# rrahn/libspm

Hardware: AMD Instinct MI355X
Metric: Gbases/s scanned, Myers k<=3 |P|=100 (higher is better)
Workload: dtype u32

## Files before the change

libspm_amd/csrc/filter.hpp:

```cpp
#pragma once

#include "brute.hpp"
#include "common.hpp"
#include "filter_shared.hpp"
#include "pack.hpp"
#include "hd.hpp"

namespace spm_hip
{

struct survivor
{
    uint32_t key;
    uint32_t t_lo, t_hi;
    uint32_t pad;
};
constexpr uint32_t kSurvInvalid = 0xFFFFFFFFu;

struct band_rec
{
    uint32_t slot;
    uint32_t val;
    uint32_t seg;
    uint32_t band;
// ... 256 lines not shown
            uint32_t wu = w[0], pu = prev[0];
#pragma unroll
            for (int q = 1; q < NWD; ++q)
                if (u == q) {
                    wu = w[q];
                    pu = prev[q];
                }
            key = (d == 16 ? wu : alignbit(wu, pu, (uint32_t)(2 * d) & 31u)) & kmask;
            const uint64_t wpos = PK ? gbase + (uint64_t)(u >> 2) * 4096 + (uint64_t)lane * 64 + (uint64_t)(u & 3) * 16
                                     : gbase + (uint64_t)u * 1024 + (uint64_t)lane * 16;
            const int64_t ts = (int64_t)wpos - 16 + d;
            if (ts >= (int64_t)P.lo && (uint64_t)ts + P.key_len <= P.hi) {
                t = (uint64_t)ts;
                has = true;
            }
        }
        emit_survivors(P, has, key, t, lane, lds);
    }
}



__device__ __forceinline__ uint32_t anchor_select(uint32_t w, uint32_t prev, uint32_t c, uint32_t cm)
{
    const uint32_t C0 = (c & 3u) * 0x55555555u, M0 = (cm & 3u) * 0x55555555u;
    const uint32_t C1 = (c >> 2) * 0x55555555u, M1 = (cm >> 2) * 0x55555555u;
    const uint32_t X = alignbit(w, prev, 2);
    const uint32_t Y = alignbit(w, prev, 4);
    uint32_t t = ((X ^ C0) & M0) | ((Y ^ C1) & M1);
    t |= t >> 1;
    return ~t & 0x55555555u;
}

template <int NWD>
__device__ __forceinline__ void filter_words_anchored(const filter_params &P, const uint32_t (&w)[NWD], const uint32_t (&prev)[NWD],
                                                      uint64_t gbase, uint32_t lane, const uint32_t *lds)
{
    static_assert(NWD % 2 == 0 || NWD == 1, "words are taken in pairs");
    const uint16_t *fp_tab = reinterpret_cast<const uint16_t *>(lds);
    const uint16_t *disp_tab = reinterpret_cast<const uint16_t *>(reinterpret_cast<const uint8_t *>(lds) + P.chd_disp_off);
#pragma unroll
    for (int j = 0; j < NWD; j += 2) {
        uint32_t todo = anchor_select(w[j], prev[j], P.anchor_c, P.anchor_cm);
        if (j + 1 < NWD)
            todo |= anchor_select(w[j + 1 < NWD ? j + 1 : j], prev[j + 1 < NWD ? j + 1 : j], P.anchor_c, P.anchor_cm) << 1;
        while (__ballot(todo != 0) != 0) {
            const bool act = todo != 0;
            const uint32_t b = act ? (uint32_t)__ffs(todo) - 1u : 0u;
            todo &= todo - 1;
            const uint32_t u = b & 1u, d = (b >> 1) + 1u;
            const uint32_t wu = (j + 1 < NWD && u) ? w[j + 1 < NWD ? j + 1 : j] : w[j];
            const uint32_t pu = (j + 1 < NWD && u) ? prev[j + 1 < NWD ? j + 1 : j] : prev[j];
            const uint32_t key = (uint32_t)((((uint64_t)wu << 32) | pu) >> (2 * d));
            const uint32_t x = chd_hash(key).x;
            const uint32_t dsp = disp_tab[x >> P.chd_bucket_shift];
            const uint32_t slot = ((x >> 3) + dsp * ((key | 1u) & 0xFFFFFFu)) & P.chd_slot_mask;
            const uint32_t f = fp_tab[slot];
            const bool hit = act && ((f ^ key ^ (key >> 16)) & 0xFFFFu) == 0;
            if (__ballot(hit) != 0) {
                if (__builtin_amdgcn_readfirstlane(cand_chunk_of(P, lds)[5]) != 0)
                    return;
                const uint64_t wpos = gbase + (uint64_t)(j + u) * 1024 + (uint64_t)lane * 16;
                const int64_t ts = (int64_t)wpos - 16 + (int64_t)d;
                const bool has = hit && ts >= (int64_t)P.lo && (uint64_t)ts + P.key_len <= P.hi;
                emit_survivors(P, has, key, has ? (uint64_t)ts : 0, lane, lds);
            }
        }
    }
}


__device__ __forceinline__ void stream_stage(const filter_params &P, uint32_t *lds)
{
    for (uint32_t i = threadIdx.x; i < P.lds_words; i += blockDim.x)
        lds[i] = P.bitmap[i];
    if ((threadIdx.x & 63) == 0) {
        uint32_t *ck = lds + P.lds_words + kCandLdsSlot + kCandRec * (threadIdx.x >> 6);
        for (uint32_t i = 0; i < kCandRec; ++i)
            ck[i] = 0;
    }
    __syncthreads();
}

enum class span_draw
{
    run,
    idle,
    done,
};

__device__ __forceinline__ span_draw draw_span(const filter_params &P, uint32_t *lds, uint32_t lane, uint32_t wave_in_wg,
                                               uint32_t waves_per_wg, uint64_t n_spans, uint64_t &sp)
{
    if (P.dynamic == 1) {
        unsigned long long t = 0;
        if (lane == 0)
            t = atomicAdd(&P.counters[kCntSpanHead], 1ull);
        sp = uniform_u64(t);
        return sp >= n_spans ? span_draw::done : span_draw::run;
    }
    __syncthreads();
    if (threadIdx.x == 0) {
        const unsigned long long t = atomicAdd(&P.counters[kCntSpanHead], (unsigned long long)waves_per_wg);
        lds[P.lds_words] = (uint32_t)t;
        lds[P.lds_words + 1] = (uint32_t)(t >> 32);
    }
    __syncthreads();
    const uint64_t base = uniform_u64(((uint64_t)lds[P.lds_words + 1] << 32) | lds[P.lds_words]);
    if (base >= n_spans)
        return span_draw::done;
    sp = base + wave_in_wg;
    return sp >= n_spans ? span_draw::idle : span_draw::run;
}

template <int SIG>
__device__ __forceinline__ uint32_t span_carry_in(const filter_params &P, uint64_t span_base, uint32_t lane, uint32_t &carry_n)
{
    uint32_t carry_in = 0;
    carry_n = 0;
    if (span_base >= 16 && lane == 0) {
        const uint4 before = load_text16(P.text, span_base - 16, P.hi);
        carry_in = pack16_sig<SIG>(before, carry_n);
    }
    carry_n = __builtin_amdgcn_readfirstlane(carry_n);
    return __builtin_amdgcn_readfirstlane(carry_in);
}

__device__ __forceinline__ uint32_t span_carry_in(const filter_params &P, uint64_t span_base, uint32_t lane)
{
    uint32_t no_n;
    return span_carry_in<4>(P, span_base, lane, no_n);
}

__device__ __forceinline__ void pack_with_prev(const uint4 &cur, uint32_t lane, uint32_t &carry_in, uint32_t &w, uint32_t &prev)
{
    w = pack16(cur);
    prev = __builtin_amdgcn_update_dpp(0u, w, 0x138 , 0xF, 0xF, false);
    if (lane == 0)
        prev = carry_in;
    carry_in = __builtin_amdgcn_readlane(w, 63);
}

template <int S, int UU, int HV, int SIG, bool KM, bool AN = false>
__device__ __forceinline__ void filter_group(const filter_params &P, const uint4 (&cur)[UU], uint64_t gbase,
                                             uint32_t &carry_in, uint32_t &carry_n, uint32_t lane,
                                             const uint32_t *lds, uint32_t idx_mask)
{
    uint32_t w[UU], prev[UU];
    uint32_t nv[SIG != 4 ? UU : 1];
#pragma unroll
    for (int u = 0; u < UU; ++u) {
        if constexpr (SIG == 4) {
            pack_with_prev(cur[u], lane, carry_in, w[u], prev[u]);
        } else {
            uint32_t nm = 0;
            w[u] = pack16_sig<SIG>(cur[u], nm);
            prev[u] = __builtin_amdgcn_update_dpp(0u, w[u], 0x138 , 0xF, 0xF, false);
            if (lane == 0)
                prev[u] = carry_in;
            carry_in = __builtin_amdgcn_readlane(w[u], 63);
            uint32_t np = __builtin_amdgcn_update_dpp(0u, nm, 0x138, 0xF, 0xF, false);
            if (lane == 0)
                np = carry_n;
            carry_n = __builtin_amdgcn_readlane(nm, 63);
            nv[u] = (nm << 16) | np;
        }
    }
    if constexpr (AN)
        filter_words_anchored<UU>(P, w, prev, gbase, lane, lds);
    else
        filter_words<S, UU, HV, SIG, false, KM>(P, w, prev, nv, gbase, lane, lds, idx_mask);
}

template <int S, int U, int HV, int SIG, bool KM, bool AN = false>
__global__ __launch_bounds__(((S == 1 && !KM && SIG == 4) || (S == 2 && U == 2)) ? 1024 : 512) void seed_filter_kernel(const filter_params P)
{
    extern __shared__ uint32_t lds[];
    stream_stage(P, lds);

    const uint32_t lane = threadIdx.x & 63;
    const uint32_t waves_per_wg = blockDim.x >> 6;
    const uint32_t wave_in_wg = (uint32_t)__builtin_amdgcn_readfirstlane(threadIdx.x >> 6);
    const uint32_t idx_mask = P.bitmap_words * 32 - 1;

    const stream_geometry G = stream_geometry_of(P.lo, P.hi, 1024, P.span_chunks);
    const uint64_t span = P.span_chunks;
    const uint8_t *lane_text = P.text + G.base0 + (uint64_t)lane * 16;

    uint64_t sp;
    for (;;) {
        const span_draw drawn = draw_span(P, lds, lane, wave_in_wg, waves_per_wg, G.n_spans, sp);
        if (drawn == span_draw::done)
            break;
        if (drawn == span_draw::idle)
            continue;
        const uint64_t c_begin = sp * span;
        const uint64_t c_end = c_begin + span < G.n_chunks ? c_begin + span : G.n_chunks;
        span_open(P, lds, lane, G.base0 + c_begin * 1024);
        uint32_t carry_n;
        uint32_t carry_in = span_carry_in<SIG>(P, G.base0 + c_begin * 1024, lane, carry_n);
        uint64_t ch = c_begin;
        const uint64_t whole_end = c_end < G.n_whole ? c_end : G.n_whole;
        const uint64_t fast_end = c_begin + (whole_end > c_begin ? (whole_end - c_begin) / U * U : 0);
        if (ch < fast_end) {
            uint4 nxt[U];
#pragma unroll
            for (int u = 0; u < U; ++u)
                nxt[u] = load16_stream(lane_text + (ch + u) * 1024);
            for (; ch < fast_end; ch += U) {
                uint4 cur[U];
#pragma unroll
                for (int u = 0; u < U; ++u)
                    cur[u] = nxt[u];
                const bool more = ch + U < fast_end;
                const uint64_t pf = more ? ch + U : ch;
                const uint64_t ustride = more ? 1024 : 0;
#pragma unroll
                for (int u = 0; u < U; ++u)
                    nxt[u] = load16_stream(lane_text + pf * 1024 + (uint64_t)u * ustride);
                if constexpr (S <= 2)
                    __builtin_amdgcn_sched_barrier(0);
                filter_group<S, U, HV, SIG, KM, AN>(P, cur, G.base0 + ch * 1024, carry_in, carry_n, lane, lds, idx_mask);
            }
        }
        for (; ch < c_end; ++ch) {
            uint4 one[1];
            one[0] = load_text16(P.text, (G.base0 + ch * 1024) | ((uint64_t)lane * 16), P.hi);
            filter_group<S, 1, HV, SIG, KM, AN>(P, one, G.base0 + ch * 1024, carry_in, carry_n, lane, lds, idx_mask);
        }
    }
    surv_close(P, cand_chunk_of(P, lds), lane);
}

constexpr uint32_t kDenseQueueCap = 192;
constexpr int kDenseBatches = 3;

template <int NP>
__device__ __forceinline__ uint32_t dense_select(const filter_params &P, uint32_t w, uint32_t prev)
{
    const uint32_t X = alignbit(w, prev, 2);
    const uint32_t Y = alignbit(w, prev, 4);
    uint32_t sel = 0;
#pragma unroll
    for (int i = 0; i < NP; ++i) {
        const uint32_t C0 = (P.pat_c[i] & 3u) * 0x55555555u, M0 = (P.pat_cm[i] & 3u) * 0x55555555u;
        const uint32_t C1 = (P.pat_c[i] >> 2) * 0x55555555u, M1 = (P.pat_cm[i] >> 2) * 0x55555555u;
        uint32_t t = ((X ^ C0) & M0) | ((Y ^ C1) & M1);
        t |= t >> 1;
        sel |= ~t;
    }
    return sel & 0x55555555u;
}

struct dense_queue
{
    uint32_t key[kDenseQueueCap];
    uint32_t off[kDenseQueueCap];
};

__device__ __forceinline__ void dense_drain(const filter_params &P, dense_queue &Q, uint32_t &qn, bool all, uint64_t span_base,
                                            uint32_t lane, const uint32_t *lds)
{
    while (qn >= 64 || (all && qn != 0)) {
        const uint32_t nb_full = qn >> 6;
        uint32_t nb = all ? (qn + 63) >> 6 : nb_full;
        nb = nb > (uint32_t)kDenseBatches ? (uint32_t)kDenseBatches : nb;
        uint32_t key[kDenseBatches], off[kDenseBatches];
        uint4 bk[kDenseBatches];
        bool v[kDenseBatches];
#pragma unroll
        for (int b = 0; b < kDenseBatches; ++b) {
            const int32_t e = (int32_t)qn - 64 * b - 1 - (int32_t)lane;
            v[b] = (uint32_t)b < nb && e >= 0;
            key[b] = 0;
            off[b] = 0;
            bk[b] = make_uint4(0, 0, 0, 0);
            if (v[b]) {
                key[b] = Q.key[e];
                off[b] = Q.off[e];
                bk[b] = P.buckets[dense_bucket(key[b], P.bucket_shift)];
            }
        }
        qn = qn > 64 * nb ? qn - 64 * nb : 0;
#pragma unroll
        for (int b = 0; b < kDenseBatches; ++b) {
            if ((uint32_t)b >= nb)
                break;
            const uint32_t f2 = dense_fp(key[b]) * 0x00010001u;
            const uint32_t x0 = bk[b].x ^ f2, x1 = bk[b].y ^ f2, x2 = bk[b].z ^ f2, x3 = bk[b].w ^ f2;
            const uint32_t z = ((x0 - 0x00010001u) & ~x0) | ((x1 - 0x00010001u) & ~x1) | ((x2 - 0x00010001u) & ~x2) |
                               ((x3 - 0x00010001u) & ~x3);
            const bool hit = v[b] && ((z & 0x80008000u) != 0 || (bk[b].w >> 16) == kDenseAcceptAll);
            if (__ballot(hit) != 0) {
                if (__builtin_amdgcn_readfirstlane(cand_chunk_of(P, lds)[5]) == 0) {
                    const int64_t ts = (int64_t)span_base + (int64_t)off[b] - 16;
                    const bool has = hit && ts >= (int64_t)P.lo && (uint64_t)ts + P.key_len <= P.hi;
                    emit_survivors(P, has, key[b], has ? (uint64_t)ts : 0, lane, lds);
                }
            }
        }
    }
}

template <int UU, int NP, int S, bool KM>
__device__ __forceinline__ void dense_group(const filter_params &P, const uint4 (&cur)[UU], uint64_t gbase, uint64_t span_base,
                                            uint32_t &carry_in, uint32_t lane, const uint32_t *lds, dense_queue &Q, uint32_t &qn)
{
    static_assert(UU % 2 == 0 || UU == 1, "words are taken in pairs");
    uint32_t w[UU], prev[UU];
#pragma unroll
    for (int u = 0; u < UU; ++u)
        pack_with_prev(cur[u], lane, carry_in, w[u], prev[u]);
    const uint32_t goff = (uint32_t)(gbase - span_base) + lane * 16;
#pragma unroll
    for (int j = 0; j < UU; j += 2) {
        constexpr bool pair = UU > 1;
        const uint32_t w0 = w[j], p0 = prev[j], w1 = w[pair ? j + 1 : j], p1 = prev[pair ? j + 1 : j];
        const uint32_t kmask = KM ? P.key_mask : 0xFFFFFFFFu;
        static_assert(kDenseBloomBits == 20, "the word address below takes bits 5..19 of the index");
        uint32_t pm = 0;
        if constexpr (S == 0) {
            uint32_t todo = dense_select<NP>(P, w0, p0);
            if (pair)
                todo |= dense_select<NP>(P, w1, p1) << 1;
            while (todo != 0) {
                const uint32_t b = (uint32_t)__ffs(todo) - 1u;
                todo &= todo - 1;
                const bool odd = (b & 1u) != 0;
                const uint64_t both = ((uint64_t)(odd ? w1 : w0) << 32) | (odd ? p1 : p0);
                const uint32_t key = (uint32_t)(both >> ((b & ~1u) + 2u));
                const uint32_t h = key ^ (key >> 13);
                const uint32_t word = *reinterpret_cast<const uint32_t *>(reinterpret_cast<const uint8_t *>(lds) + ((h >> 3) & 0x1FFFCu));
                pm |= __builtin_amdgcn_ubfe(word, h, 1) << b;
            }
        } else {
#pragma unroll
            for (int u = 0; u < (pair ? 2 : 1); ++u) {
#pragma unroll
                for (int d = S; d <= 16; d += S) {
                    const uint32_t wu = u ? w1 : w0, pu = u ? p1 : p0;
                    const uint32_t key = (d == 16 ? wu : alignbit(wu, pu, (2 * d) & 31)) & kmask;
                    const uint32_t h = key ^ (key >> 13);
                    const uint32_t word = *reinterpret_cast<const uint32_t *>(reinterpret_cast<const uint8_t *>(lds) + ((h >> 3) & 0x1FFFCu));
                    pm |= __builtin_amdgcn_ubfe(word, h, 1) << (2 * (d - 1) + u);
                }
            }
        }
        while (__ballot(pm != 0) != 0) {
            const bool pos = pm != 0;
            const uint32_t b = pos ? (uint32_t)__ffs(pm) - 1u : 0u;
            pm &= pm - 1;
            const bool odd = (b & 1u) != 0;
            const uint64_t both = ((uint64_t)(odd ? w1 : w0) << 32) | (odd ? p1 : p0);
            const uint32_t key = (uint32_t)(both >> ((b & ~1u) + 2u)) & kmask;
            const uint64_t mm = __ballot(pos);
            if (pos) {
                const uint32_t q = qn + __popcll(mm & ((1ull << lane) - 1));
                Q.key[q] = key;
                Q.off[q] = goff + (uint32_t)j * 1024u + (odd ? 1024u : 0u) + (b >> 1) + 1u;
            }
            qn += __popcll(mm);
            queue_sync();
            if (qn > kDenseQueueCap - 64)
                dense_drain(P, Q, qn, false, span_base, lane, lds);
        }
    }
}

template <int U, int NP, int S = 0, bool KM = false>
__global__ __launch_bounds__(1024) void seed_filter_dense_kernel(const filter_params P)
{
    extern __shared__ uint32_t lds[];
    stream_stage(P, lds);

    const uint32_t lane = threadIdx.x & 63;
    const uint32_t waves_per_wg = blockDim.x >> 6;
    const uint32_t wave_in_wg = (uint32_t)__builtin_amdgcn_readfirstlane(threadIdx.x >> 6);
    dense_queue &Q = *reinterpret_cast<dense_queue *>(lds + P.lds_words + kCandLdsSlot + kCandRec * 16 +
                                                      (sizeof(dense_queue) / 4) * wave_in_wg);
    uint32_t qn = 0;

    const stream_geometry G = stream_geometry_of(P.lo, P.hi, 1024, P.span_chunks);
    const uint64_t span = P.span_chunks;
    const uint8_t *lane_text = P.text + G.base0 + (uint64_t)lane * 16;

    uint64_t sp;
    for (;;) {
        const span_draw drawn = draw_span(P, lds, lane, wave_in_wg, waves_per_wg, G.n_spans, sp);
        if (drawn == span_draw::done)
            break;
        if (drawn == span_draw::idle)
            continue;
        const uint64_t c_begin = sp * span;
        const uint64_t c_end = c_begin + span < G.n_chunks ? c_begin + span : G.n_chunks;
        const uint64_t span_base = G.base0 + c_begin * 1024;
        span_open(P, lds, lane, span_base);
        uint32_t carry_in = span_carry_in(P, span_base, lane);
        uint64_t ch = c_begin;
        const uint64_t whole_end = c_end < G.n_whole ? c_end : G.n_whole;
        const uint64_t fast_end = c_begin + (whole_end > c_begin ? (whole_end - c_begin) / U * U : 0);
        if (ch < fast_end) {
            uint4 nxt[U];
#pragma unroll
            for (int u = 0; u < U; ++u)
                nxt[u] = load16_stream(lane_text + (ch + u) * 1024);
            for (; ch < fast_end; ch += U) {
                uint4 cur[U];
#pragma unroll
                for (int u = 0; u < U; ++u)
                    cur[u] = nxt[u];
                const bool more = ch + U < fast_end;
                const uint64_t pf = more ? ch + U : ch;
                const uint64_t ustride = more ? 1024 : 0;
#pragma unroll
                for (int u = 0; u < U; ++u)
                    nxt[u] = load16_stream(lane_text + pf * 1024 + (uint64_t)u * ustride);
                __builtin_amdgcn_sched_barrier(0);
                dense_group<U, NP, S, KM>(P, cur, G.base0 + ch * 1024, span_base, carry_in, lane, lds, Q, qn);
            }
        }
        for (; ch < c_end; ++ch) {
            uint4 one[1];
            one[0] = load_text16(P.text, G.base0 + ch * 1024 + (uint64_t)lane * 16, P.hi);
            dense_group<1, NP, S, KM>(P, one, G.base0 + ch * 1024, span_base, carry_in, lane, lds, Q, qn);
        }
        dense_drain(P, Q, qn, true, span_base, lane, lds);
    }
    surv_close(P, cand_chunk_of(P, lds), lane);
}

template <int S, int U2, int HV, bool KM>
__global__ __launch_bounds__(1024) void seed_filter_packed_kernel(const filter_params P, const uint4 *__restrict__ shadow)
{
    extern __shared__ uint32_t lds[];
    stream_stage(P, lds);

    constexpr int NWD = 4 * U2;
    const uint32_t lane = threadIdx.x & 63;
    const uint32_t waves_per_wg = blockDim.x >> 6;
    const uint32_t wave_in_wg = (uint32_t)__builtin_amdgcn_readfirstlane(threadIdx.x >> 6);
    const uint32_t idx_mask = P.bitmap_words * 32 - 1;

    const stream_geometry G = stream_geometry_of(P.lo, P.hi, 4096, P.span_chunks);
    const uint64_t span = P.span_chunks;
    const uint4 *lane_src = shadow + (G.base0 / 64) + lane;

    uint64_t sp;
    for (;;) {
        const span_draw drawn = draw_span(P, lds, lane, wave_in_wg, waves_per_wg, G.n_spans, sp);
        if (drawn == span_draw::done)
            break;
        if (drawn == span_draw::idle)
            continue;
        const uint64_t c_begin = sp * span;
        const uint64_t c_end = c_begin + span < G.n_chunks ? c_begin + span : G.n_chunks;
        const uint64_t fast_end = c_begin + (c_end - c_begin + U2 - 1) / U2 * U2;
        span_open(P, lds, lane, G.base0 + c_begin * 4096);
        uint32_t carry_in = 0;
        {
            const uint64_t first_word = (G.base0 + c_begin * 4096) / 16;
            if (first_word > 0 && lane == 0)
                carry_in = reinterpret_cast<const uint32_t *>(shadow)[first_word - 1];
            carry_in = __builtin_amdgcn_readfirstlane(carry_in);
        }
        uint4 nxt[U2];
#pragma unroll
        for (int u = 0; u < U2; ++u)
            nxt[u] = load16_stream(reinterpret_cast<const uint8_t *>(lane_src + (c_begin + u) * 64));
        for (uint64_t ch = c_begin; ch < fast_end; ch += U2) {
            uint4 cur[U2];
#pragma unroll
            for (int u = 0; u < U2; ++u)
                cur[u] = nxt[u];
            const bool more = ch + U2 < fast_end;
            const uint64_t pf = more ? ch + U2 : ch;
            const uint64_t ustride = more ? 64 : 0;
#pragma unroll
            for (int u = 0; u < U2; ++u)
                nxt[u] = load16_stream(reinterpret_cast<const uint8_t *>(lane_src + pf * 64 + (uint64_t)u * ustride));
            __builtin_amdgcn_sched_barrier(0);
            uint32_t w[NWD], prev[NWD];
            const uint32_t nv[1] = {0};
#pragma unroll
            for (int u = 0; u < U2; ++u) {
                w[4 * u + 0] = cur[u].x;
                w[4 * u + 1] = cur[u].y;
                w[4 * u + 2] = cur[u].z;
                w[4 * u + 3] = cur[u].w;
                uint32_t p0 = __builtin_amdgcn_update_dpp(0u, cur[u].w, 0x138 , 0xF, 0xF, false);
                if (lane == 0)
                    p0 = carry_in;
                carry_in = __builtin_amdgcn_readlane(cur[u].w, 63);
                prev[4 * u + 0] = p0;
                prev[4 * u + 1] = cur[u].x;
                prev[4 * u + 2] = cur[u].y;
                prev[4 * u + 3] = cur[u].z;
            }
            filter_words<S, NWD, HV, 4, true, KM>(P, w, prev, nv, G.base0 + ch * 4096, lane, lds, idx_mask);
        }
    }
    surv_close(P, cand_chunk_of(P, lds), lane);
}

struct verify_params
{
    const uint8_t *text;
    uint64_t text_alloc;
    uint64_t ctx_begin;
    uint64_t scan_begin;
    uint64_t scan_end;
    uint64_t pos_offset;
    const band_rec *bands;
    const unsigned long long *counters;
    uint32_t band_counter;
    uint32_t preselected;
    uint64_t band_cap;
    ulonglong2 *band_tab;
    uint32_t table_mask, band_bits;
    uint32_t runs;
    const uint8_t *surplus;
    uint32_t Bw;
    uint32_t overlap;
    uint32_t max_m;
    const uint32_t *peq32;
    uint32_t sigma;
    uint32_t nw_table;
    uint32_t max_k;
    const int32_t *m;
    const int32_t *k;
    uint32_t report_begin;
    uint32_t max_span;
    uint32_t wave_text;
    unsigned long long *seen;
    uint32_t seen_mask;
    spm_hit *hits;
    unsigned long long *hit_counter;
    uint64_t hit_cap;
    unsigned long long *overflow;
    const uint64_t *seg_offsets;
    uint64_t n_segments;
    const uint32_t *seg_owned;
};

struct resolve_params
{
    const survivor *surv;
    unsigned long long *counters;
    uint64_t surv_cap;
    const pass_entry *passes;
    const uint4 *entries;
    uint32_t key_len;
    uint32_t flank_check;
    uint32_t pieces_check;
    const uint8_t *text;
    uint64_t text_alloc;
    const uint8_t *needle_ranks;
    const uint32_t *needle_offsets;
    const uint16_t *seed_q;
    const int32_t *m, *k;
    uint64_t hay_begin, hay_end;
    const uint64_t *seg_offsets;
    uint64_t n_segments;
    uint32_t Bw, overlap, max_m;
    uint32_t band_bits;
    ulonglong2 *band_tab;
    uint32_t table_mask;
    band_rec *bands;
    uint64_t band_cap;
    const uint32_t *needle_pk;
    const uint32_t *pk_offsets;
    uint32_t exact_hits;
    uint32_t report_begin;
    uint64_t scan_begin, scan_end;
    uint64_t pos_offset;
    const uint32_t *seg_owned;
    unsigned long long *seen;
    uint32_t seen_mask;
    spm_hit *hits;
    unsigned long long *hit_counter, *overflow;
    uint64_t hit_cap;
    uint32_t *table_poison;
};

__device__ __forceinline__ unsigned long long band_value(unsigned long long stored, bool counting)
{
    return counting ? (unsigned long long)(uint32_t)(stored + 1ull) : ~stored;
}
__device__ __forceinline__ void band_release(ulonglong2 *tab, uint32_t slot)
{
    tab[slot] = make_ulonglong2(kBandEmpty, ~0ull);
}

__device__ __forceinline__ uint4 load_bytes16(const uint8_t *p)
{
    uint4 v;
    __builtin_memcpy(&v, p, 16);
    return v;
}

__device__ __forceinline__ uint4 load_bytes16_guarded(const uint8_t *base, uint64_t idx, uint64_t limit)
{
    if (idx + 16 <= limit)
        return load_bytes16(base + idx);
    uint32_t w[4] = {0xFFFFFFFFu, 0xFFFFFFFFu, 0xFFFFFFFFu, 0xFFFFFFFFu};
    for (int b = 0; b < 16; ++b)
        if (idx + b < limit)
            w[b >> 2] = (w[b >> 2] & ~(0xFFu << (8 * (b & 3)))) | ((uint32_t)base[idx + b] << (8 * (b & 3)));
    return make_uint4(w[0], w[1], w[2], w[3]);
}

__device__ __forceinline__ uint32_t diff16(const uint4 a, const uint4 b, uint32_t n)
{
    const uint32_t d[4] = {a.x ^ b.x, a.y ^ b.y, a.z ^ b.z, a.w ^ b.w};
    uint32_t r = 0;
#pragma unroll
    for (uint32_t i = 0; i < 4; ++i) {
        const uint32_t have = n > 4 * i ? n - 4 * i : 0;
        const uint32_t mask = have >= 4 ? 0xFFFFFFFFu : (have == 0 ? 0u : (1u << (8 * have)) - 1);
        r |= d[i] & mask;
    }
    return r;
}

__device__ __forceinline__ bool seed_intact(const resolve_params &P, uint64_t t, uint32_t val, uint32_t r, uint32_t q_whole,
                                            int64_t hay_b, int64_t hay_e)
{
    if (!P.needle_ranks)
        return true;
    const uint32_t pat = val >> 11, x = val & 0x7FF;
    struct
    {
        uint32_t q;
    } sp{q_whole ? q_whole : P.seed_q[pat]};
    const uint32_t o = x - r;
    const int64_t ts = (int64_t)t - (int64_t)r;
    if (ts < hay_b || ts + (int64_t)sp.q > hay_e)
        return false;
    const uint8_t *nd = P.needle_ranks + P.needle_offsets[pat] + o;
    for (uint32_t i = 0; i < sp.q; i += 16) {
        const uint32_t n = sp.q - i < 16 ? sp.q - i : 16;
        if (diff16(load_bytes16_guarded(P.text, (uint64_t)ts + i, P.text_alloc), load_bytes16(nd + i), n))
            return false;
    }
    return true;
}

constexpr uint32_t kPieceRoundsShift = 21, kPieceMissingShift = 28;

__device__ __forceinline__ bool pieces_apply(const resolve_params &P, uint64_t t, uint32_t val, uint32_t m, uint32_t k, int64_t hay_b,
                                             int64_t hay_e)
{
    if (!P.pieces_check || k == 0 || k > 7 || m < 32)
        return false;
    const int64_t d = (int64_t)t - (int64_t)(val & 0x7FF);
    return d - (int64_t)k >= hay_b && d + (int64_t)(m + k) <= hay_e;
}

__device__ __forceinline__ uint32_t pieces_visit(const resolve_params &P, uint64_t t, uint32_t val, uint32_t &rng, uint32_t m, uint32_t k)
{
    const uint32_t pat = val >> 11, x = val & 0x7FF;
    const uint32_t n_rounds = m >> 4;
    uint32_t done = (rng >> kPieceRoundsShift) & 0x7F, missing = (rng >> kPieceMissingShift) & 7;
// ... 1126 lines not shown
```

Before: 6463.

## Batch dense survivor enqueue with a wave prefix sum and pair the bloom probes

The per-pair ballot loop that appended one hit per lane per iteration is replaced. Each lane now gathers presence masks for all word pairs, counts its hits, and uses a DPP wave prefix sum to get its write offset into the queue. All hits are then written in bulk, in chunks bounded by the remaining queue room. The S==0 selection loop also probes two candidate positions per iteration to expose more LDS-load parallelism. This is meant to cut the ballot and queue_sync rounds per group and keep lanes from idling on uneven hit counts, at the cost of more registers for the held masks and a more complex chunked drain loop.

```diff
diff --git a/libspm_amd/csrc/filter.hpp b/libspm_amd/csrc/filter.hpp
--- a/libspm_amd/csrc/filter.hpp
+++ b/libspm_amd/csrc/filter.hpp
@@ -582,36 +582,61 @@
     }
 }
 
+__device__ __forceinline__ uint32_t wave_prefix_sum(uint32_t v)
+{
+    v += __builtin_amdgcn_update_dpp(0u, v, 0x111 , 0xF, 0xF, false);
+    v += __builtin_amdgcn_update_dpp(0u, v, 0x112 , 0xF, 0xF, false);
+    v += __builtin_amdgcn_update_dpp(0u, v, 0x114 , 0xF, 0xF, false);
+    v += __builtin_amdgcn_update_dpp(0u, v, 0x118 , 0xF, 0xF, false);
+    v += __builtin_amdgcn_update_dpp(0u, v, 0x142 , 0xA, 0xF, false);
+    v += __builtin_amdgcn_update_dpp(0u, v, 0x143 , 0xC, 0xF, false);
+    return v;
+}
+
+__device__ __forceinline__ uint32_t dense_pair_key(uint32_t w0, uint32_t p0, uint32_t w1, uint32_t p1, uint32_t b)
+{
+    const bool odd = (b & 1u) != 0;
+    const uint64_t both = ((uint64_t)(odd ? w1 : w0) << 32) | (odd ? p1 : p0);
+    return (uint32_t)(both >> ((b & ~1u) + 2u));
+}
+
+__device__ __forceinline__ uint32_t dense_presence_word(const uint32_t *lds, uint32_t h)
+{
+    static_assert(kDenseBloomBits == 20, "the word address takes bits 5..19 of the index");
+    return *reinterpret_cast<const uint32_t *>(reinterpret_cast<const uint8_t *>(lds) + ((h >> 3) & 0x1FFFCu));
+}
+
 template <int UU, int NP, int S, bool KM>
 __device__ __forceinline__ void dense_group(const filter_params &P, const uint4 (&cur)[UU], uint64_t gbase, uint64_t span_base,
                                             uint32_t &carry_in, uint32_t lane, const uint32_t *lds, dense_queue &Q, uint32_t &qn)
 {
     static_assert(UU % 2 == 0 || UU == 1, "words are taken in pairs");
+    constexpr bool pair = UU > 1;
+    constexpr int NPM = pair ? UU / 2 : 1;
     uint32_t w[UU], prev[UU];
 #pragma unroll
     for (int u = 0; u < UU; ++u)
         pack_with_prev(cur[u], lane, carry_in, w[u], prev[u]);
     const uint32_t goff = (uint32_t)(gbase - span_base) + lane * 16;
+    const uint32_t kmask = KM ? P.key_mask : 0xFFFFFFFFu;
+    uint32_t pmv[NPM];
 #pragma unroll
     for (int j = 0; j < UU; j += 2) {
-        constexpr bool pair = UU > 1;
         const uint32_t w0 = w[j], p0 = prev[j], w1 = w[pair ? j + 1 : j], p1 = prev[pair ? j + 1 : j];
-        const uint32_t kmask = KM ? P.key_mask : 0xFFFFFFFFu;
-        static_assert(kDenseBloomBits == 20, "the word address below takes bits 5..19 of the index");
-        uint32_t pm = 0;
+        uint32_t m = 0;
         if constexpr (S == 0) {
             uint32_t todo = dense_select<NP>(P, w0, p0);
             if (pair)
                 todo |= dense_select<NP>(P, w1, p1) << 1;
             while (todo != 0) {
-                const uint32_t b = (uint32_t)__ffs(todo) - 1u;
+                const uint32_t b0 = (uint32_t)__ffs(todo) - 1u;
                 todo &= todo - 1;
-                const bool odd = (b & 1u) != 0;
-                const uint64_t both = ((uint64_t)(odd ? w1 : w0) << 32) | (odd ? p1 : p0);
-                const uint32_t key = (uint32_t)(both >> ((b & ~1u) + 2u));
-                const uint32_t h = key ^ (key >> 13);
-                const uint32_t word = *reinterpret_cast<const uint32_t *>(reinterpret_cast<const uint8_t *>(lds) + ((h >> 3) & 0x1FFFCu));
-                pm |= __builtin_amdgcn_ubfe(word, h, 1) << b;
+                const uint32_t b1 = todo != 0 ? (uint32_t)__ffs(todo) - 1u : b0;
+                todo &= todo - 1;
+                const uint32_t key0 = dense_pair_key(w0, p0, w1, p1, b0), key1 = dense_pair_key(w0, p0, w1, p1, b1);
+                const uint32_t h0 = key0 ^ (key0 >> 13), h1 = key1 ^ (key1 >> 13);
+                const uint32_t word0 = dense_presence_word(lds, h0), word1 = dense_presence_word(lds, h1);
+                m |= (__builtin_amdgcn_ubfe(word0, h0, 1) << b0) | (__builtin_amdgcn_ubfe(word1, h1, 1) << b1);
             }
         } else {
 #pragma unroll
@@ -621,23 +646,54 @@
                     const uint32_t wu = u ? w1 : w0, pu = u ? p1 : p0;
                     const uint32_t key = (d == 16 ? wu : alignbit(wu, pu, (2 * d) & 31)) & kmask;
                     const uint32_t h = key ^ (key >> 13);
-                    const uint32_t word = *reinterpret_cast<const uint32_t *>(reinterpret_cast<const uint8_t *>(lds) + ((h >> 3) & 0x1FFFCu));
-                    pm |= __builtin_amdgcn_ubfe(word, h, 1) << (2 * (d - 1) + u);
+                    m |= __builtin_amdgcn_ubfe(dense_presence_word(lds, h), h, 1) << (2 * (d - 1) + u);
                 }
             }
         }
+        pmv[j / 2] = m;
+    }
+    if constexpr (pair) {
+        uint32_t cnt = 0;
+#pragma unroll
+        for (int i = 0; i < NPM; ++i)
+            cnt += __popc(pmv[i]);
+        uint32_t incl = wave_prefix_sum(cnt);
+        uint32_t r = incl - cnt;
+        for (;;) {
+            const uint32_t left = __builtin_amdgcn_readlane(incl, 63);
+            if (left == 0)
+                break;
+            const uint32_t room = kDenseQueueCap - qn;
+            const uint32_t n = left < room ? left : room;
+#pragma unroll
+            for (int i = 0; i < NPM; ++i) {
+                while (pmv[i] != 0 && r < n) {
+                    const uint32_t b = (uint32_t)__ffs(pmv[i]) - 1u;
+                    pmv[i] &= pmv[i] - 1;
+                    Q.key[qn + r] = dense_pair_key(w[2 * i], prev[2 * i], w[2 * i + 1], prev[2 * i + 1], b) & kmask;
+                    Q.off[qn + r] = goff + (uint32_t)i * 2048u + ((b & 1u) << 10) + (b >> 1) + 1u;
+                    ++r;
+                }
+            }
+            qn += n;
+            r -= n;
+            incl -= n;
+            asm volatile("" : "+v"(r), "+v"(incl));
+            queue_sync();
+            if (qn > kDenseQueueCap - 64)
+                dense_drain(P, Q, qn, false, span_base, lane, lds);
+        }
+    } else {
+        uint32_t pm = pmv[0];
         while (__ballot(pm != 0) != 0) {
             const bool pos = pm != 0;
             const uint32_t b = pos ? (uint32_t)__ffs(pm) - 1u : 0u;
             pm &= pm - 1;
-            const bool odd = (b & 1u) != 0;
-            const uint64_t both = ((uint64_t)(odd ? w1 : w0) << 32) | (odd ? p1 : p0);
-            const uint32_t key = (uint32_t)(both >> ((b & ~1u) + 2u)) & kmask;
             const uint64_t mm = __ballot(pos);
             if (pos) {
                 const uint32_t q = qn + __popcll(mm & ((1ull << lane) - 1));
-                Q.key[q] = key;
-                Q.off[q] = goff + (uint32_t)j * 1024u + (odd ? 1024u : 0u) + (b >> 1) + 1u;
+                Q.key[q] = dense_pair_key(w[0], prev[0], w[0], prev[0], b) & kmask;
+                Q.off[q] = goff + (b >> 1) + 1u;
             }
             qn += __popcll(mm);
             queue_sync();
```

Measured after the change: 6465 (median of 3 runs). Within noise of the previous version (+0.0%).
